# floe/backscrub

Hardware: AMD Instinct MI355X
Metric: composited frames/sec at 640×480 (batch), 1/2/4/8 MI355X + mask IoU vs CPU ref (higher is better)
Workload: dtype f32 (network) / u8 (image kernels); 1 GPU; BASELINE configs[1]: batch=256 640x480 frames, segm_lite_v681.tflite; moving scene: ring of 4 batches, a new one every step; 1 step = prep+network+decode+mask+blend, inputs resident in HBM; streams_per_gpu=256, library=bsx 0.1 (HIP gfx950, f32 NHWC)

## Files before the change

### backscrub_amd/csrc/kernels_seg.hip

```cpp
#ifndef __HIPCC_RTC__
#include <hip/hip_runtime.h>
#endif
#ifndef BSX_SEG_RTC
#include "debug_switches.hpp"

#include <algorithm>
#include <cstdlib>
#include <type_traits>

#include "kernels.hpp"
#include "mfma_tile.hpp"
#include "segments.hpp"
#endif

#if defined(BSX_SEG_RTC)
#define BSX_SEG_D(T, NAME) constexpr T d = kSeg##NAME; (void)d_rt
#elif defined(BSX_SEG_PROBE)
#define BSX_SEG_D(T, NAME) constexpr T d = kProbe##NAME; (void)d_rt
#else
#define BSX_SEG_D(T, NAME) const T& d = d_rt
#endif

namespace bsx {
#ifdef BSX_SEG_RTC
// ... 285 lines not shown
  for (int s = 0; s < 7; s++) {
    const int k = 4 * s + g;
    const bool valid = k < 27;
    const int fy = k / 9, r9 = k - 9 * fy, fx = r9 / 3, ci = r9 - 3 * fx;
    koff[s] = valid ? fy * rowf + fx * 3 + ci : 0;
    ws[s] = valid ? (w + d.stem.w_off)[(unsigned)(k * d.stem.cout_pad + li)] : 0.f;
  }
  const float4 bias_s = ld4(w + d.stem.b_off + cq4);
  const Clamp cl_stem = clamp_of(d.stem.act), cl_pw = clamp_of(d.pw.act), cl_dw = clamp_of(d.dw.act);
  const int ntile = AR * ctiles;
  const int xe = li;
  __syncthreads();

  float* x_f = a_t;
  float wr[4];
  load_wtile(wr, w, d.pw, 0, li, g);
  const float4 bias_p = ld4(w + d.pw.b_off + cq4);
  float4 sumA = f4zero();
  auto stem_pw_epilogue = [&](const f4acc acc, const RowTile rt) {
    float4 v = acc_quad(acc);
    const int x2 = 16 * rt.ct + xe, gy = ar0 + rt.row, gx = ac0 + x2;
    v = f4add(v, bias_s);
    v = STEM_HSWISH ? hswish4(v) : clamp4(v, cl_stem);
    f4acc pa = {0.f, 0.f, 0.f, 0.f};
    if (!(d.dbg_skip & 2)) {
      pa = __builtin_amdgcn_mfma_f32_16x16x4f32(wr[0], v.x, pa, 0, 0, 0);
      pa = __builtin_amdgcn_mfma_f32_16x16x4f32(wr[1], v.y, pa, 0, 0, 0);
      pa = __builtin_amdgcn_mfma_f32_16x16x4f32(wr[2], v.z, pa, 0, 0, 0);
      pa = __builtin_amdgcn_mfma_f32_16x16x4f32(wr[3], v.w, pa, 0, 0, 0);
    }
    if (x2 < AC) {
      const bool row_owned = gy >= max(2 * r0, 0) && gy < min(2 * r0 + 2 * d.TR, d.H1);
      if (row_owned && gx >= 2 * c0 && gx < min(2 * c0 + 2 * d.TC, d.W1)) {
        stg4<H16>(A_out, (unsigned)((gy * d.W1 + gx) * 16 + cq4), v);
        sumA = f4add(sumA, v);
      }
      float4 xv = acc_quad(pa);
      const bool inside = gy >= 0 && gy < d.H1 && gx >= 0 && gx < d.W1;
      xv = inside ? clamp4(f4add(xv, bias_p), cl_pw) : f4zero();
      st4(x_f + (rt.row * AC + x2) * 16 + cq4, xv);
    }
  };
  for (int t = wave; t < ntile && !(d.dbg_skip & 1); t += 8) {
    const bool two = t + 4 < ntile;
    const RowTile r0t = row_tile(t, ctiles, d.m_ct), r1t = row_tile(two ? t + 4 : t, ctiles, d.m_ct);
    const float* base0 = in_t + (2 * r0t.row) * rowf + 6 * min(16 * r0t.ct + li, AC - 1);
    const float* base1 = in_t + (2 * r1t.row) * rowf + 6 * min(16 * r1t.ct + li, AC - 1);
    float av0[7], av1[7];
#pragma unroll
    for (int s7 = 0; s7 < 7; s7++) { av0[s7] = base0[koff[s7]]; av1[s7] = base1[koff[s7]]; }
    f4acc acc0 = {0.f, 0.f, 0.f, 0.f}, acc1 = {0.f, 0.f, 0.f, 0.f};
#pragma unroll
    for (int s7 = 0; s7 < 7; s7++) {
      acc0 = __builtin_amdgcn_mfma_f32_16x16x4f32(ws[s7], av0[s7], acc0, 0, 0, 0);
      acc1 = __builtin_amdgcn_mfma_f32_16x16x4f32(ws[s7], av1[s7], acc1, 0, 0, 0);
    }
    stem_pw_epilogue(acc0, r0t);
    if (two) stem_pw_epilogue(acc1, r1t);
  }
  const int quad = lane & 3, px = lane >> 2;
  f4v wd[9];
#pragma unroll
  for (int k = 0; k < 9; k++) wd[k] = ldv(w + d.dw.w_off + k * 16 + 4 * quad);
  const f4v bias_d = ldv(w + d.dw.b_off + 4 * quad);
  const int cox[3] = {(2 * px) * 16 + 4 * quad, (2 * px + 1) * 16 + 4 * quad, (2 * px + 2) * 16 + 4 * quad};
  __syncthreads();

  float4 sumB = f4zero();
  for (int py = wave; py < d.TR && !(d.dbg_skip & 4); py += 4) {
    if (r0 + py >= d.H2) break;
    if (px < d.TC && c0 + px < d.W2) {
      const float4 v = clamp4(tof4(dw3x3(x_f, AC * 16, 2 * py, cox, wd) + bias_d), cl_dw);
      stg4<H16>(b0_out, (unsigned)(((r0 + py) * d.W2 + c0 + px) * 16 + 4 * quad), v);
      sumB = f4add(sumB, v);
    }
  }
  float* s_red = in_t;
  wave_reduce16<0>(sumA, s_red, wave, lane);
  wave_reduce16<1>(sumB, s_red + 256, wave, lane);
  __syncthreads();
  store_partials(s_red, fa + d.part_a_off + (long)t_ * 16);
  store_partials(s_red + 256, fa + d.part_b0_off + (long)t_ * 16);
}

#ifdef BSX_SEG_RTC
extern "C" __global__ __launch_bounds__(kSegThreads) __attribute__((amdgpu_waves_per_eu(6, 6))) void bsx_seg_k2(
#else
template <bool H16>
__global__ __launch_bounds__(kSegThreads) __attribute__((amdgpu_waves_per_eu(6, 6))) void seg_k2_k(
#endif
    const SegK2 d_rt, float* __restrict__ arena, long per_frame, const float* __restrict__ w, int n_frames) {
  BSX_SEG_D(SegK2, K2);
  unsigned f_, t_;
  xcd_frame_tile((unsigned)(d.tiles_y * d.tiles_x), (unsigned)n_frames, &f_, &t_);
  const int f = (int)f_, ty = (int)t_ / d.tiles_x, tx = (int)t_ - ty * d.tiles_x;
  const int r0 = ty * d.TR, c0 = tx * d.TC;
  const int BR = 2 * d.TR + 1, BC = 2 * d.TC + 1, br0 = 2 * r0 - d.dw_pt, bc0 = 2 * c0 - d.dw_pl, RW = d.rw, ctiles = RW >> 4;
  float* fa = arena + (size_t)f * (size_t)per_frame;
  float* B_t = seg_smem + kScrFloats;
  float* x_t = B_t + BR * RW * 16;
  const float* b0_in = fa + d.b0_off;
  float* B_out = fa + d.B_off;
  float* c0_out = fa + d.c0_off;
  const int tid = threadIdx.x, lane = tid & 63, wave = wave_uniform(tid >> 6), li = lane & 15, g = lane >> 4, cq4 = 4 * g;
  const int ntile = BR * ctiles, xe = li;
  const int la = col_a(li, g), lb = col_b(li, g, RW >> 1);
  constexpr int kB0 = 6;
  float4 b0v[kB0];
#pragma unroll
  for (int j = 0; j < kB0; j++) {
    const int t = wave + 4 * j;
    b0v[j] = f4zero();
    if (t < ntile) {
      const RowTile rt = row_tile(t, ctiles, d.m_ct);
      const int gy = br0 + rt.row, gx = bc0 + 16 * rt.ct + li;
      if (gy >= 0 && gy < d.H2 && gx >= 0 && gx < d.W2) b0v[j] = ldg4<H16>(b0_in, (unsigned)((gy * d.W2 + gx) * 16 + 4 * g));
    }
  }
  seg_gate(d.gate, fa, w, seg_smem, B_t);
  const float4 sv = ld4(seg_smem + kScrGate + 4 * g);
  float wr[4];
  load_wtile(wr, w, d.pw_a, 0, li, g);
  const float4 bias_a = ld4(w + d.pw_a.b_off + cq4);
  const Clamp cl_a = clamp_of(d.pw_a.act), cl_b = clamp_of(d.pw_b.act), cl_dw = clamp_of(d.dw.act);

  float4 sumB = f4zero();
#pragma unroll
  for (int j = 0; j < kB0; j++) {
    const int t = wave + 4 * j;
    if (t >= ntile) break;
    const RowTile rt = row_tile(t, ctiles, d.m_ct);
    float4 a = b0v[j];
    a = make_float4(__fmul_rn(a.x, sv.x), __fmul_rn(a.y, sv.y), __fmul_rn(a.z, sv.z), __fmul_rn(a.w, sv.w));
    const f4acc acc = mma16(a, wr);
    float4 v = acc_quad(acc);
    const int x2 = 16 * rt.ct + xe, hy = br0 + rt.row, hx = bc0 + x2;
    if (x2 < BC) {
      v = clamp4(f4add(v, bias_a), cl_a);
      st4(B_t + (rt.row * RW + 16 * rt.ct) * 16 + la, v);
      const bool row_owned = hy >= max(2 * r0, 0) && hy < min(2 * r0 + 2 * d.TR, d.H2);
      if (row_owned && hx >= 2 * c0 && hx < min(2 * c0 + 2 * d.TC, d.W2)) {
        stg4<H16>(B_out, (unsigned)((hy * d.W2 + hx) * 16 + cq4), v);
        sumB = f4add(sumB, v);
      }
    }
  }
  float* s_red = seg_smem + kScrRed;
  wave_reduce16<0>(sumB, s_red, wave, lane);
  __syncthreads();
  store_partials(s_red, fa + d.part_B_off + (long)t_ * 16);

  const int C = d.dw.C, ngrp = (C + 15) >> 4, quad = lane & 3, px = lane >> 2;
  const int cox[3] = {col_b(2 * px, quad, RW >> 1), col_b(2 * px + 1, quad, RW >> 1), col_b(2 * px + 2, quad, RW >> 1)};
  for (int grp = 0; grp < ngrp && !(d.dbg_skip & 2); grp++) {
    load_wtile(wr, w, d.pw_b, 16 * grp, li, g);
    const float4 bias_b = ld4(w + d.pw_b.b_off + 16 * grp + cq4);
    for (int t = wave; t < ntile; t += 4) {
      const RowTile rt = row_tile(t, ctiles, d.m_ct);
      const f4acc acc = mma16(ld4(B_t + (rt.row * RW + 16 * rt.ct) * 16 + la), wr);
      float4 v = acc_quad(acc);
      const int x2 = 16 * rt.ct + xe, hy = br0 + rt.row, hx = bc0 + x2;
      if (x2 < BC) {
        const bool inside = hy >= 0 && hy < d.H2 && hx >= 0 && hx < d.W2;
        v = inside ? clamp4(f4add(v, bias_b), cl_b) : f4zero();
        st4(x_t + (rt.row * RW + 8 * rt.ct) * 16 + lb, v);
      }
    }
    const int ch = 16 * grp + 4 * quad;
    f4v wd[9];
    f4v bias_d = {0.f, 0.f, 0.f, 0.f};
    if (ch < C) {
#pragma unroll
      for (int k = 0; k < 9; k++) wd[k] = ldv(w + d.dw.w_off + (unsigned)(k * C + ch));
      bias_d = ldv(w + d.dw.b_off + ch);
    }
    __syncthreads();
    if (ch < C && px < d.TC && c0 + px < d.W3)
      for (int py = wave; py < d.TR && r0 + py < d.H3; py += 4) {
        const float4 v = clamp4(tof4(dw3x3(x_t, RW * 16, 2 * py, cox, wd) + bias_d), cl_dw);
        stg4<H16>(c0_out, (unsigned)(((r0 + py) * d.W3 + c0 + px) * C + ch), v);
      }
    __syncthreads();
  }
}

constexpr int kGatedRows = 5;
constexpr int kLoStride = kSegLoStride;
struct GatedPre { float4 s[kGatedRows]; int ly0, lx0, LC; };
template <bool H16>
__device__ __forceinline__ GatedPre gated_prefetch(const float* __restrict__ skip, const float* __restrict__ lo, int H, int W, int HL, int WL, bool half_pixel,
                                                   float hs, float wsc, int r0, int c0, int ZH, int ZC, float* l_t) {
  const int tid = threadIdx.x, lane = tid & 63, wave = wave_uniform(tid >> 6), li = lane & 15, g = lane >> 4;
  GatedPre pre;
  const int ix = c0 - 1 + li;
  const bool col_in = li < ZC && ix >= 0 && ix < W;
#pragma unroll
  for (int j = 0; j < kGatedRows; j++) {
    const int zy = wave + 4 * j, iy = r0 - 1 + zy;
    pre.s[j] = f4zero();
    if (zy < ZH && iy >= 0 && iy < H && col_in) pre.s[j] = ldg4<H16>(skip, (unsigned)((iy * W + ix) * 16 + 4 * g));
  }
  int ly0, ly1, lx0, lx1, t0, t1;
  float fr;
  up_axis(max(r0 - 1, 0), hs, half_pixel, HL, &ly0, &t1, &fr);
  up_axis(min(r0 - 2 + ZH, H - 1), hs, half_pixel, HL, &t0, &ly1, &fr);
  up_axis(max(c0 - 1, 0), wsc, half_pixel, WL, &lx0, &t1, &fr);
  up_axis(min(c0 - 2 + ZC, W - 1), wsc, half_pixel, WL, &t0, &lx1, &fr);
  const int LR = ly1 - ly0 + 1, LC = lx1 - lx0 + 1;
  pre.ly0 = ly0; pre.lx0 = lx0; pre.LC = LC;
  float4 v[3];
#pragma unroll
  for (int j = 0; j < 3; j++) {
    const int ly = wave + 4 * j;
    v[j] = f4zero();
    if (ly < LR && lane < LC * 4) v[j] = ldg4<H16>(lo, (unsigned)(((ly0 + ly) * WL + lx0 + (lane >> 2)) * 16 + 4 * (lane & 3)));
  }
#pragma unroll
  for (int j = 0; j < 3; j++) {
    const int ly = wave + 4 * j;
    if (ly < LR && lane < LC * 4) st4(l_t + ly * LC * kLoStride + col_l(lane >> 2, lane & 3), v[j]);
  }
  return pre;
}
__device__ __forceinline__ void gated_compute(const GatedPre& pre, const float* l_t, int H, int W, int HL, int WL, bool half_pixel, float hs, float wsc, const float* s_gate,
                                              const SegConvW& pw, const float* __restrict__ w, int r0, int c0, int ZH, int ZC, float* z_t) {
  const int tid = threadIdx.x, lane = tid & 63, wave = wave_uniform(tid >> 6), li = lane & 15, g = lane >> 4, cq4 = 4 * g;
  float wr[4];
  load_wtile(wr, w, pw, 0, li, g);
  const float4 bias = ld4(w + pw.b_off + cq4);
  const float4 gv = ld4(s_gate + 4 * g);
  const Clamp cl = clamp_of(pw.act);
  const int ix = c0 - 1 + li;
  int x0, x1;
  float dx;
  up_axis(min(max(ix, 0), W - 1), wsc, half_pixel, WL, &x0, &x1, &dx);
  const int xo0 = col_l(x0 - pre.lx0, g), xo1 = col_l(x1 - pre.lx0, g);
  const int xe = li;
  const bool ecol_in = xe < ZC && ix >= 0 && ix < W;
#pragma unroll
  for (int j = 0; j < kGatedRows; j++) {
    const int zy = wave + 4 * j, iy = r0 - 1 + zy;
    if (zy >= ZH) break;
    const bool row_in = iy >= 0 && iy < H;
    int y0, y1;
    float dy;
    up_axis(min(max(iy, 0), H - 1), hs, half_pixel, HL, &y0, &y1, &dy);
    const float* l0 = l_t + (y0 - pre.ly0) * pre.LC * kLoStride;
    const float* l1 = l_t + (y1 - pre.ly0) * pre.LC * kLoStride;
    const float4 ta = ld4(l0 + xo0), tb = ld4(l1 + xo0), tc = ld4(l0 + xo1), td = ld4(l1 + xo1);
    const float w00 = (1.f - dy) * (1.f - dx), w10 = dy * (1.f - dx), w01 = (1.f - dy) * dx, w11 = dy * dx;
    const float4 sk = pre.s[j];
    float4 a;
    a.x = fmaf(sk.x, gv.x, fmaf(td.x, w11, fmaf(tc.x, w01, fmaf(tb.x, w10, ta.x * w00))));
    a.y = fmaf(sk.y, gv.y, fmaf(td.y, w11, fmaf(tc.y, w01, fmaf(tb.y, w10, ta.y * w00))));
    a.z = fmaf(sk.z, gv.z, fmaf(td.z, w11, fmaf(tc.z, w01, fmaf(tb.z, w10, ta.z * w00))));
    a.w = fmaf(sk.w, gv.w, fmaf(td.w, w11, fmaf(tc.w, w01, fmaf(tb.w, w10, ta.w * w00))));
    const f4acc acc = mma16(a, wr);
    float4 v = acc_quad(acc);
    v = (ecol_in && row_in) ? clamp4(f4add(v, bias), cl) : f4zero();
    if (xe < ZC) st4(z_t + zy * 256 + col_a(xe, g), v);
  }
}

#ifdef BSX_SEG_RTC
extern "C" __global__ __launch_bounds__(kSegThreads) void bsx_seg_k3(
#else
template <bool H16>
__global__ __launch_bounds__(kSegThreads) void seg_k3_k(
#endif
    const SegK3 d_rt, float* __restrict__ arena, long per_frame, const float* __restrict__ w, int n_frames) {
  BSX_SEG_D(SegK3, K3);
  unsigned f_, t_;
  xcd_frame_tile((unsigned)(d.tiles_y * d.tiles_x), (unsigned)n_frames, &f_, &t_);
  const int f = (int)f_, ty = (int)t_ / d.tiles_x, tx = (int)t_ - ty * d.tiles_x;
  const int r0 = ty * d.TR, c0 = tx * d.TC, ZH = d.TR + 2, ZC = d.TC + 2;
  float* fa = arena + (size_t)f * (size_t)per_frame;
  float* z_t = seg_smem + kScrFloats;
  float* l_t = z_t + ZH * 256;
  float* lo_out = fa + d.lo_off;
  const int tid = threadIdx.x, lane = tid & 63, wave = wave_uniform(tid >> 6), li = lane & 15, g = lane >> 4, cq4 = 4 * g;
  const GatedPre pre = gated_prefetch<H16>(fa + d.skip_off, fa + d.lo2_off, d.H2, d.W2, d.HL, d.WL, d.half_pixel != 0, d.hs, d.ws, r0, c0, ZH, ZC, l_t);
  if (tid < 16) seg_smem[kScrGate + tid] = fa[d.g_off + tid];
  __syncthreads();
  gated_compute(pre, l_t, d.H2, d.W2, d.HL, d.WL, d.half_pixel != 0, d.hs, d.ws, seg_smem + kScrGate, d.pw1, w, r0, c0, ZH, ZC, z_t);
  const int pc = min(li, 13);
  const int coz[3] = {col_a(pc, g), col_a(pc + 1, g), col_a(pc + 2, g)};
  f4v wd[9];
#pragma unroll
  for (int k = 0; k < 9; k++) wd[k] = ldv(w + d.dw.w_off + k * 16 + cq4);
  const f4v bias_d = ldv(w + d.dw.b_off + cq4);
  const Clamp cl_dw = clamp_of(d.dw.act), cl_2 = clamp_of(d.pw2.act);
  float wr[4];
  load_wtile(wr, w, d.pw2, 0, li, g);
  const float4 bias2 = ld4(w + d.pw2.b_off + cq4);
  __syncthreads();
  float4 sum = f4zero();
  const int xe = li;
  for (int py = wave; py < d.TR && r0 + py < d.H2; py += 4) {
    const f4v zc = ldv(z_t + (py + 1) * 256 + coz[1]);
    const float4 dv = clamp4(tof4(dw3x3(z_t, 256, py, coz, wd) + bias_d), cl_dw);
    const f4acc acc = mma16(f4add(dv, tof4(zc)), wr);
    float4 v = acc_quad(acc);
    if (xe < d.TC && c0 + xe < d.W2) {
      v = clamp4(f4add(v, bias2), cl_2);
      stg4<H16>(lo_out, (unsigned)(((r0 + py) * d.W2 + c0 + xe) * 16 + cq4), v);
      sum = f4add(sum, v);
    }
  }
  float* s_red = seg_smem + kScrRed;
  wave_reduce16<0>(sum, s_red, wave, lane);
  __syncthreads();
  store_partials(s_red, fa + d.part_lo_off + (long)t_ * 16);
}

#ifdef BSX_SEG_RTC
extern "C" __global__ __launch_bounds__(kSegThreads) __attribute__((amdgpu_waves_per_eu(5, 5))) void bsx_seg_tail(
#else
template <int CO, bool LOGITS, bool SIGMOID, bool H16>
__global__ __launch_bounds__(kSegThreads) __attribute__((amdgpu_waves_per_eu(5, 5))) void seg_tail_k(
#endif
    const SegTail d_rt, float* __restrict__ arena, long per_frame, float* __restrict__ net_out,
                                                          uint8_t* __restrict__ ofinal, const float* __restrict__ w, int n_frames, const int* __restrict__ slot_of) {
  BSX_SEG_D(SegTail, TAIL);
  unsigned f_, t_;
  xcd_frame_tile((unsigned)(d.tiles_y * d.tiles_x), (unsigned)n_frames, &f_, &t_);
  const int f = (int)f_, ty = (int)t_ / d.tiles_x, tx = (int)t_ - ty * d.tiles_x;
  const int r0 = ty * d.TR, c0 = tx * d.TC, ZH = d.TR + 2, ZC = d.TC + 2;
  float* fa = arena + (size_t)f * (size_t)per_frame;
  float* z_t = seg_smem + kScrFloats;
  float* l_t = z_t + max(ZH * 256, kGateStageFloats);
  uint8_t* of = ofinal + (size_t)(slot_of ? slot_of[f] : f) * (size_t)(d.H0 * d.W0);
  float* no = net_out + (size_t)f * (size_t)(d.H0 * d.W0 * CO);
  const int tid = threadIdx.x, lane = tid & 63, wave = wave_uniform(tid >> 6), li = lane & 15, g = lane >> 4, cq4 = 4 * g;
  const int fy = g >> 1, fx = g & 1, ix = c0 + li;
  const GatedPre pre = gated_prefetch<H16>(fa + d.skip_off, fa + d.lo_off, d.H1, d.W1, d.HL, d.WL, d.half_pixel != 0, d.hs, d.ws, r0, c0, ZH, ZC, l_t);
  constexpr int kRowsB = 5;
// ... 143 lines not shown
```

### backscrub_amd/csrc/plan.cpp

```cpp
#include "debug_switches.hpp"
#include "plan.hpp"
#include "gen_seg.hpp"
#include "gen_mid.hpp"

#include <algorithm>
#include <cmath>
#include <cstdio>
#include <cstdlib>
#include <cstring>
#include <map>

namespace bsx {
namespace {

void conv_geometry(int in, int k, int s, int d, bool same, int* out, int* pad) {
  int eff = (k - 1) * d + 1;
  *out = same ? (in + s - 1) / s : (in + s - eff) / s;
  int total = (*out - 1) * s + eff - in;
  *pad = total > 0 ? total / 2 : 0;
}

uint16_t f32_to_f16_rn(float f) {
  uint32_t x; memcpy(&x, &f, 4);
  const uint32_t sign = (x >> 16) & 0x8000u;
// ... 445 lines not shown
      if ((m.kind == (int)StepKind::PwConv && m.gemv) || m.kind == kMicroTail || m.kind == (int)StepKind::Conv) return;
    lower_frame_program(g, plan, steps, ext, part_n, part_hw, 64, policy);
    if (plan->program.empty()) lower_frame_program(g, plan, steps, ext, part_n, part_hw, kLdsScratchFloats, policy);
  };
  if (const char* force = BSX_DBG_ENV("BSX_PLAN_POLICY")) { plan->program_policy = (unsigned)atoi(force) & 7u; lower(plan->program_policy); plan->program_arena_bytes = program_arena_bytes(*plan); return; }
  unsigned best = 0;
  long best_b = -1;
  for (unsigned pol = 0; pol < 8; pol++) {
    lower(pol);
    if (plan->program.empty()) continue;
    const long b = program_arena_bytes(*plan);
    if (best_b < 0 || b < best_b) { best_b = b; best = pol; }
  }
  lower(best);
  plan->program_policy = best;
  plan->program_arena_bytes = program_arena_bytes(*plan);
}

std::string verify_program_lds(const Plan& plan) {
  const auto& b = plan.program_blocks;
  for (size_t i = 0; i < b.size(); i++) {
    if (b[i].off < plan.program_scratch_floats || b[i].off + b[i].len > plan.lds_zero_off() || b[i].len <= 0 || b[i].from > b[i].until)
      return "block out of range: " + b[i].what;
    for (size_t j = i + 1; j < b.size(); j++) {
      const bool time = b[i].from <= b[j].until && b[j].from <= b[i].until;
      const bool mem = b[i].off < b[j].off + b[j].len && b[j].off < b[i].off + b[i].len;
      if (time && mem) return "overlap: " + b[i].what + " [" + std::to_string(b[i].from) + "," + std::to_string(b[i].until) + "] and " + b[j].what + " [" +
                              std::to_string(b[j].from) + "," + std::to_string(b[j].until) + "]";
    }
  }
  for (const MicroOp& m : plan.program) {
    for (const Loc* l : {&m.in0, &m.in1, &m.in2, &m.res, &m.scale, &m.out})
      if (l->space == kLocLds && (l->off < plan.program_scratch_floats || l->off >= plan.program_lds_floats)) return "operand outside the LDS block area";
    if (m.stage_floats > 0 && (m.w_lds < plan.program_scratch_floats || m.w_lds + m.stage_floats > plan.program_lds_floats)) return "weight slot outside the LDS block area";
  }
  return "ok";
}


namespace {

bool resize_weights_uniform(int in, int out, bool align, bool half_pixel) {
  std::vector<double> wsum(in, 0.0);
  const float scale = (align && out > 1) ? (float)(in - 1) / (float)(out - 1) : (float)in / (float)out;
  for (int o = 0; o < out; o++) {
    const float v = half_pixel ? ((float)o + 0.5f) * scale - 0.5f : (float)o * scale;
    const float fl = std::floor(v);
    const int lo = std::max((int)fl, 0), hi = std::min((int)std::ceil(v), in - 1);
    const float frac = v - (float)lo;
    wsum[lo] += 1.0 - frac; wsum[hi] += frac;
  }
  const double want = (double)out / (double)in;
  for (double x : wsum) if (std::fabs(x - want) > 1e-5) return false;
  return true;
}

SegConvW conv_w(const Step& st) { SegConvW c; c.w_off = (long long)st.w_off; c.b_off = (long long)st.b_off; c.Cin = st.kh * st.kw * st.Cin; c.Cout = st.Cout; c.cout_pad = st.cout_pad; c.act = st.act; return c; }
SegDwW dw_w(const Step& st) { SegDwW c; c.w_off = (long long)st.w_off; c.b_off = (long long)st.b_off; c.C = st.Cout; c.act = st.act; return c; }
SegFc fc_w(const Step& st) { SegFc c; c.w_off = (long long)st.w2_off; c.b_off = (long long)st.b_off; c.Cin = st.Cin; c.Cout = st.Cout; c.act = st.act; return c; }

bool is_pw16(const Step& st) { return st.kind == StepKind::PwConv && st.Cin == 16 && st.Cout == 16 && st.cout_pad == 16 && st.OH * st.OW > 4; }
bool is_fc_step(const Step& st) { return st.kind == StepKind::PwConv && st.OH * st.OW == 1 && st.w2_off != 0 && st.residual < 0 && st.in_scale < 0 && st.in2 < 0 && st.Cin <= 32 && st.Cin % 8 == 0 && st.Cout <= 32; }
bool is_dw3(const Step& st, int stride) {
  return st.kind == StepKind::DwConv && st.kh == 3 && st.kw == 3 && st.sh == stride && st.sw == stride && st.dh == 1 && st.dw == 1;
}
int tiles_for(int extent, int target) { return (extent + target - 1) / target; }

}

static bool seg_fail(int where) { if (BSX_DBG_ENV("BSX_SEG_DEBUG")) fprintf(stderr, "segmentation: check %d failed\n", where); return false; }
static bool build_segments(Graph& g, Plan* plan) {
  const std::vector<Step>& S = plan->steps;
  const int NS = (int)S.size();
  if (NS < 9 + 15) return seg_fail(1);
  auto uses_of = [&](int t) {
    int n = 0;
    for (const Step& q : S) {
      for (int u : {q.concat_in.empty() ? q.in0 : -1, q.in1, q.in2, q.residual, q.in_scale}) n += (u == t);
      for (int u : q.concat_in) n += (u == t);
    }
    return n + (t == g.output);
  };
  auto dims = [&](int t, int k) { return g.tensors[t].dims[k]; };

  const Step &stem = S[0], &hpw = S[1], &hdw = S[2];
  if (!(stem.kind == StepKind::Conv && stem.in0 == g.input && stem.kh == 3 && stem.kw == 3 && stem.sh == 2 && stem.sw == 2 && stem.dh == 1 && stem.dw == 1 &&
        stem.Cin == 3 && stem.Cout == 16 && stem.cout_pad == 16 && stem.residual < 0)) return seg_fail(2);
  const int A = stem.out;
  if (!(is_pw16(hpw) && hpw.in0 == A && hpw.residual < 0 && hpw.in_scale < 0 && hpw.in2 < 0 && uses_of(hpw.out) == 1)) return seg_fail(3);
  if (!(is_dw3(hdw, 2) && hdw.in0 == hpw.out && hdw.Cout == 16 && hdw.residual < 0)) return seg_fail(4);
  const int b0 = hdw.out;
  const Step &g1 = S[3], &f1a = S[4], &f1b = S[5], &pwa = S[6], &pwb = S[7], &kdw = S[8];
  if (!(g1.kind == StepKind::Gap && g1.concat_in.empty() && g1.in0 == b0 && is_fc_step(f1a) && f1a.in0 == g1.out && is_fc_step(f1b) && f1b.in0 == f1a.out &&
        f1a.Cin == 16 && f1b.Cout == 16 && uses_of(b0) == 2)) return seg_fail(5);
  if (!(is_pw16(pwa) && pwa.in0 == b0 && pwa.in_scale == f1b.out && pwa.residual < 0 && pwa.in2 < 0 && uses_of(f1b.out) == 1)) return seg_fail(6);
  const int B = pwa.out;
  if (!(pwb.kind == StepKind::PwConv && pwb.in0 == B && pwb.Cin == 16 && pwb.cout_pad % 16 == 0 && pwb.residual < 0 && pwb.in_scale < 0 && pwb.in2 < 0 &&
        uses_of(pwb.out) == 1 && pwb.Cout % 4 == 0)) return seg_fail(7);
  if (!(is_dw3(kdw, 2) && kdw.in0 == pwb.out && kdw.residual < 0)) return seg_fail(8);
  const int c0 = kdw.out;
  const Step &tr = S[NS - 7], &tg = S[NS - 6], &tf1 = S[NS - 5], &tf2 = S[NS - 4], &tpw = S[NS - 3], &tdw = S[NS - 2], &ttc = S[NS - 1];
  if (!(tr.kind == StepKind::Resize && tr.Cin == 16 && tr.OH == dims(A, 1) && tr.OW == dims(A, 2))) return seg_fail(9);
  const int lo = tr.in0, up = tr.out;
  auto pools = [](const Step& q, int a, int b) { return q.kind == StepKind::Gap && q.concat_in.size() == 2 && ((q.concat_in[0] == a && q.concat_in[1] == b) || (q.gap_sum && q.concat_in[0] == b && q.concat_in[1] == a)); };
  if (!(pools(tg, A, up) && is_fc_step(tf1) && tf1.in0 == tg.out &&
        is_fc_step(tf2) && tf2.in0 == tf1.out && tf2.Cout == 16)) return seg_fail(10);
  if (!(is_pw16(tpw) && tpw.in0 == A && tpw.in_scale == tf2.out && tpw.in2 == up && tpw.residual < 0)) return seg_fail(11);
  if (!(is_dw3(tdw, 1) && tdw.in0 == tpw.out && tdw.residual == tpw.out && tdw.Cout == 16 && tdw.pad_t == 1 && tdw.pad_l == 1)) return seg_fail(12);
  if (!(ttc.kind == StepKind::TConv && ttc.in0 == tdw.out && ttc.kh == 2 && ttc.kw == 2 && ttc.Cin == 16 && (ttc.Cout == 1 || ttc.Cout == 2) && ttc.out == g.output)) return seg_fail(13);
  if (uses_of(A) != 3 || uses_of(up) != 2 || uses_of(tpw.out) != 2 || uses_of(tdw.out) != 1 || uses_of(tf2.out) != 1) return seg_fail(14);
  if (!resize_weights_uniform(tr.H, tr.OH, tr.align_corners, tr.half_pixel) || !resize_weights_uniform(tr.W, tr.OW, tr.align_corners, tr.half_pixel)) return seg_fail(15);
  const Step &kr = S[NS - 14], &kg = S[NS - 13], &kf1 = S[NS - 12], &kf2 = S[NS - 11], &kp1 = S[NS - 10], &kd = S[NS - 9], &kp2 = S[NS - 8];
  if (!(kr.kind == StepKind::Resize && kr.Cin == 16 && kr.OH == dims(B, 1) && kr.OW == dims(B, 2))) return seg_fail(16);
  const int lo2 = kr.in0, up2 = kr.out;
  if (!(pools(kg, B, up2) && is_fc_step(kf1) && kf1.in0 == kg.out &&
        is_fc_step(kf2) && kf2.in0 == kf1.out && kf2.Cout == 16)) return seg_fail(17);
  if (!(is_pw16(kp1) && kp1.in0 == B && kp1.in_scale == kf2.out && kp1.in2 == up2 && kp1.residual < 0)) return seg_fail(18);
  if (!(is_dw3(kd, 1) && kd.in0 == kp1.out && kd.residual == kp1.out && kd.Cout == 16 && kd.pad_t == 1 && kd.pad_l == 1)) return seg_fail(19);
  if (!(is_pw16(kp2) && kp2.in0 == kd.out && kp2.out == lo && kp2.residual < 0 && kp2.in_scale < 0 && kp2.in2 < 0)) return seg_fail(20);
  if (uses_of(B) != 3 || uses_of(up2) != 2 || uses_of(kp1.out) != 2 || uses_of(kd.out) != 1 || uses_of(kf2.out) != 1 || uses_of(lo) != 1 || uses_of(lo2) != 1) return seg_fail(21);
  if (!resize_weights_uniform(kr.H, kr.OH, kr.align_corners, kr.half_pixel) || !resize_weights_uniform(kr.W, kr.OW, kr.align_corners, kr.half_pixel)) return seg_fail(22);
  if (uses_of(c0) != 1) return seg_fail(23);
  auto clampish = [](int a) { return a == kActNone || a == kActRelu || a == kActRelu6; };
  if (!(clampish(stem.act) || stem.act == kActHswish) || !(ttc.act == kActNone || ttc.act == kActSigmoid) || (ttc.act == kActSigmoid && ttc.Cout != 1)) return seg_fail(34);
  for (const Step* q : {&hpw, &hdw, &pwa, &pwb, &kdw, &kp1, &kd, &kp2, &tpw, &tdw}) if (!clampish(q->act)) return seg_fail(35);

  size_t top = plan->arena_floats_per_stream;
  auto reserve = [&](size_t floats) { size_t at = top; top += (floats + 63) / 64 * 64; return (long long)at; };
  auto synth = [&](const char* name, int n, int C) {
    TensorInfo t; t.dims[0] = 1; t.dims[1] = n; t.dims[2] = 1; t.dims[3] = C; t.shape = {1, n, 1, C}; t.name = name;
    g.tensors.push_back(t);
    plan->tensor_off.push_back(-1);
    return (int)g.tensors.size() - 1;
  };
  SegPlan sp;
  int tgt[8] = {4, 14, 4, 7, 16, 14, 18, 14};
  if (const char* e = BSX_DBG_ENV("BSX_SEG_TILES")) sscanf(e, "%d,%d,%d,%d,%d,%d,%d,%d", &tgt[0], &tgt[1], &tgt[2], &tgt[3], &tgt[4], &tgt[5], &tgt[6], &tgt[7]);
  auto split = [&](int extent, int target, int* tile, int* n) { *n = tiles_for(extent, std::max(1, target)); *tile = (extent + *n - 1) / *n; };

  SegHead& h = sp.head;
  h.H0 = stem.H; h.W0 = stem.W; h.H1 = stem.OH; h.W1 = stem.OW; h.H2 = hdw.OH; h.W2 = hdw.OW;
  h.stem_pt = stem.pad_t; h.stem_pl = stem.pad_l; h.dw_pt = hdw.pad_t; h.dw_pl = hdw.pad_l;
  h.stem = conv_w(stem); h.pw = conv_w(hpw); h.dw = dw_w(hdw);
  split(h.H2, tgt[0], &h.TR, &h.tiles_y); split(h.W2, tgt[1], &h.TC, &h.tiles_x);
  h.lds_floats = seg_head_lds_floats(h);
  h.rw = seg_row_width(2 * h.TC + 1); h.m_ct = (65536u + (unsigned)(h.rw / 16) - 1) / (unsigned)(h.rw / 16);
  if (h.TR > 4 || h.TC > 15 || (4 * h.TC + 3) * 3 > 192) return seg_fail(30);
  SegK2& k2 = sp.k2;
  k2.H2 = hdw.OH; k2.W2 = hdw.OW; k2.H3 = kdw.OH; k2.W3 = kdw.OW; k2.dw_pt = kdw.pad_t; k2.dw_pl = kdw.pad_l;
  k2.pw_a = conv_w(pwa); k2.pw_b = conv_w(pwb); k2.dw = dw_w(kdw);
  split(k2.H3, tgt[2], &k2.TR, &k2.tiles_y); split(k2.W3, tgt[3], &k2.TC, &k2.tiles_x);
  k2.lds_floats = seg_k2_lds_floats(k2);
  k2.rw = seg_row_width(2 * k2.TC + 1); k2.m_ct = (65536u + (unsigned)(k2.rw / 16) - 1) / (unsigned)(k2.rw / 16);
  if (k2.TC > 15 || ((2 * k2.TR + 1) * (k2.rw / 16) + 3) / 4 > 6) return seg_fail(31);
  SegK3& k3 = sp.k3;
  k3.H2 = kp1.OH; k3.W2 = kp1.OW; k3.HL = kr.H; k3.WL = kr.W; k3.half_pixel = kr.half_pixel; k3.align_corners = kr.align_corners;
  k3.pw1 = conv_w(kp1); k3.pw2 = conv_w(kp2); k3.dw = dw_w(kd);
  split(k3.H2, tgt[4], &k3.TR, &k3.tiles_y); split(k3.W2, tgt[5], &k3.TC, &k3.tiles_x);
  k3.hs = seg_up_scale(k3.HL, k3.H2, k3.align_corners != 0); k3.ws = seg_up_scale(k3.WL, k3.W2, k3.align_corners != 0);
  if (!BSX_DBG_ENV("BSX_SEG_LO_WORST")) k3.lo_floats = seg_lo_window_floats(k3.H2, k3.W2, k3.HL, k3.WL, k3.half_pixel != 0, k3.align_corners != 0, k3.TR, k3.TC, k3.tiles_y, k3.tiles_x);
  k3.lds_floats = seg_k3_lds_floats(k3);
  if (k3.TC > 14 || k3.TR > 18) return seg_fail(32);
  SegTail& tl = sp.tail;
  tl.H1 = tpw.OH; tl.W1 = tpw.OW; tl.HL = tr.H; tl.WL = tr.W; tl.H0 = ttc.OH; tl.W0 = ttc.OW; tl.half_pixel = tr.half_pixel; tl.align_corners = tr.align_corners;
  tl.pw = conv_w(tpw); tl.dw = dw_w(tdw); tl.tc_w_off = (long long)ttc.w_off; tl.tc_b_off = (long long)ttc.b_off; tl.Co = ttc.Cout; tl.act3 = ttc.act;
  split(tl.H1, tgt[6], &tl.TR, &tl.tiles_y); split(tl.W1, tgt[7], &tl.TC, &tl.tiles_x);
  tl.hs = seg_up_scale(tl.HL, tl.H1, tl.align_corners != 0); tl.ws = seg_up_scale(tl.WL, tl.W1, tl.align_corners != 0);
  if (!BSX_DBG_ENV("BSX_SEG_LO_WORST")) tl.lo_floats = seg_lo_window_floats(tl.H1, tl.W1, tl.HL, tl.WL, tl.half_pixel != 0, tl.align_corners != 0, tl.TR, tl.TC, tl.tiles_y, tl.tiles_x);
  tl.lds_floats = seg_tail_lds_floats(tl);
  if (tl.TC > 14 || tl.TR > 18) return seg_fail(33);
  const int lds_cap = 160 * 256;
  if (h.lds_floats > lds_cap || k2.lds_floats > lds_cap || k3.lds_floats > lds_cap || tl.lds_floats > lds_cap) return seg_fail(24);
  if (ttc.OH != 2 * tpw.OH || ttc.OW != 2 * tpw.OW || h.H2 != k3.H2 || h.W2 != k3.W2) return seg_fail(25);
  if (h.tiles_y * h.tiles_x > 1024 || k2.tiles_y * k2.tiles_x > 1024 || k3.tiles_y * k3.tiles_x > 1024) return seg_fail(26);

  const int pA = synth("partials(A)", h.tiles_y * h.tiles_x, 16), pb0 = synth("partials(b0)", h.tiles_y * h.tiles_x, 16);
  const int pB = synth("partials(B)", k2.tiles_y * k2.tiles_x, 16), plo = synth("partials(lo)", k3.tiles_y * k3.tiles_x, 16);
  const int pgt = BSX_DBG_ENV("BSX_SEG_NO_GATE_KERNEL") ? -1 : synth("gate(tail)", 1, 16);
  if (pgt >= 0) plan->tensor_off[pgt] = reserve(16);
  for (int t : {A, b0, B, c0, lo2, lo, kf2.out, pA, pb0, pB, plo}) plan->tensor_off[t] = reserve(g.tensors[t].elems());
  for (int t : {hpw.out, g1.out, f1a.out, f1b.out, pwb.out, up2, kg.out, kf1.out, kp1.out, kd.out, up, tg.out, tf1.out, tf2.out, tpw.out, tdw.out})
    if (t != g.output) plan->tensor_off[t] = -1;
  plan->arena_floats_per_stream = top;
  plan->seg_stored = {A, b0, B, c0, lo};

  h.a_off = plan->tensor_off[A]; h.b0_off = plan->tensor_off[b0]; h.part_a_off = plan->tensor_off[pA]; h.part_b0_off = plan->tensor_off[pb0];
  k2.b0_off = plan->tensor_off[b0]; k2.B_off = plan->tensor_off[B]; k2.c0_off = plan->tensor_off[c0]; k2.part_B_off = plan->tensor_off[pB];
  k2.gate.n_parts = 1; k2.gate.n_fc = 2; k2.gate.sum_parts = 0;
  k2.gate.part[0].off = plan->tensor_off[pb0]; k2.gate.part[0].n = h.tiles_y * h.tiles_x; k2.gate.part[0].C = 16; k2.gate.part[0].hw = (float)(h.H2 * h.W2);
  k2.gate.fc[0] = fc_w(f1a); k2.gate.fc[1] = fc_w(f1b);
  k3.skip_off = plan->tensor_off[B]; k3.lo2_off = plan->tensor_off[lo2]; k3.g_off = plan->tensor_off[kf2.out]; k3.lo_off = plan->tensor_off[lo];
  k3.part_lo_off = plan->tensor_off[plo];
  tl.skip_off = plan->tensor_off[A]; tl.lo_off = plan->tensor_off[lo];
  tl.gate.n_parts = 2; tl.gate.n_fc = 2; tl.gate.sum_parts = tg.gap_sum ? 1 : 0;
  tl.gate.part[0].off = plan->tensor_off[pA]; tl.gate.part[0].n = h.tiles_y * h.tiles_x; tl.gate.part[0].C = 16; tl.gate.part[0].hw = (float)(h.H1 * h.W1);
  tl.gate.part[1].off = plan->tensor_off[plo]; tl.gate.part[1].n = k3.tiles_y * k3.tiles_x; tl.gate.part[1].C = 16; tl.gate.part[1].hw = (float)(k3.H2 * k3.W2);
  tl.gate.fc[0] = fc_w(tf1); tl.gate.fc[1] = fc_w(tf2);
  if (BSX_DBG_ENV("BSX_SEG_GATE_SKIP")) k2.gate.timing_skip = tl.gate.timing_skip = 1;
  if (const char* e = BSX_DBG_ENV("BSX_SEG_SKIP")) sscanf(e, "%d,%d,%d,%d", &h.dbg_skip, &k2.dbg_skip, &k3.dbg_skip, &tl.dbg_skip);
  tl.pre_gate_off = pgt >= 0 ? plan->tensor_off[pgt] : -1;
  if (tl.gate.fc[0].Cin != (tl.gate.sum_parts ? 16 : 32) || k2.gate.fc[0].Cin != 16) return seg_fail(27);

  std::vector<Step> mid(S.begin() + 9, S.begin() + (NS - 14));
  Step gate = kg;
  gate.concat_in = {B, lo2};
  gate.in0 = B;
  gate.label += "*";
  mid.push_back(gate); mid.push_back(kf1); mid.push_back(kf2);
  std::map<int, int> part_n, part_hw;
  part_n[B] = k2.tiles_y * k2.tiles_x; part_hw[B] = k2.H2 * k2.W2;
  const long B_real = plan->tensor_off[B];
  plan->tensor_off[B] = plan->tensor_off[pB];
  build_frame_program(g, plan, mid, {c0, B, lo2, kf2.out}, part_n, part_hw);
  plan->tensor_off[B] = B_real;
  if (plan->program.empty()) return seg_fail(28);
  sp.on = true;
  plan->seg = sp;
#ifdef BSX_DEBUG_SWITCHES
  if (const char* path = BSX_DBG_ENV("BSX_SEG_DUMP")) {
    if (FILE* f = fopen(path, "w")) { fputs(seg_constants_text(sp, "kProbe").c_str(), f); fclose(f); }
  }
#endif
  char line[256];
  plan->seg_text.clear();
  auto add = [&](const char* name, int TR, int TC, int ty, int tx, int lds, std::initializer_list<int> stores) {
    snprintf(line, sizeof line, "segment %-5s tile %dx%d, %dx%d tiles per frame, LDS %.1f KiB, stores", name, TR, TC, ty, tx, lds / 256.0);
    plan->seg_text += line;
    for (int t : stores) plan->seg_text += " t" + std::to_string(t);
    plan->seg_text += stores.size() ? "\n" : " the network output\n";
  };
  add("head", h.TR, h.TC, h.tiles_y, h.tiles_x, h.lds_floats, {A, b0}); add("k2", k2.TR, k2.TC, k2.tiles_y, k2.tiles_x, k2.lds_floats, {B, c0});
  add("k3", k3.TR, k3.TC, k3.tiles_y, k3.tiles_x, k3.lds_floats, {lo}); add("tail", tl.TR, tl.TC, tl.tiles_y, tl.tiles_x, tl.lds_floats, {});
  return true;
}


MidGeometry mid_geometry_default() {
  static const MidGeometry geo = [] {
    MidGeometry m{kFrameThreads, kLdsTotalFloats};
    if (const char* e = BSX_DBG_ENV("BSX_MID_LANES")) { const int v = atoi(e); if (v == 512 || v == 1024) m.lanes = v; }
    if (const char* e = BSX_DBG_ENV("BSX_MID_LDS_KB")) { const int v = atoi(e); if (v >= 64 && v <= 160) m.lds_floats = v * 256; }
    return m;
  }();
  return geo;
}

bool build_plan(const Graph& g_in, Plan* plan, std::string* err, bool reuse_arena, bool segments) {
  auto fail = [&](const std::string& m) { if (err) *err = m; return false; };
  { const MidGeometry geo = mid_geometry_default(); plan->mid_lanes = geo.lanes; plan->lds_total_floats = geo.lds_floats; }
  Graph g = g_in;
  int NT = (int)g.tensors.size();
  const int NN = (int)g.nodes.size();

  std::vector<std::vector<int>> users(NT);
  for (int i = 0; i < NN; i++) for (int t : g.nodes[i].inputs) if (t >= 0 && !g.tensors[t].is_const) users[t].push_back(i);
  auto single_user = [&](int t) -> int { return (t != g.output && users[t].size() == 1) ? users[t][0] : -1; };

  std::vector<char> fused(NN, 0);
  std::vector<Step> steps;
  std::vector<float>& W = plan->weights;
  W.clear();
  auto align_w = [&]() { while (W.size() % 4) W.push_back(0.f); };

  for (int i = 0; i < NN; i++) {
    if (fused[i]) continue;
    const Node& n = g.nodes[i];
    const TensorInfo& out_t = g.tensors[n.output];
    Step st;
    st.last_node = n.index;
    auto T = [&](int k) -> const TensorInfo& { return g.tensors[n.inputs[k]]; };

    auto chain_epilogue = [&](int cur) -> int {
      for (;;) {
        int u = single_user(cur);
        if (u < 0 || fused[u]) break;
        const Node& y = g.nodes[u];
        if (is_unary(y.type) && st.act == kActNone && st.residual < 0) {
          st.act = unary_act(y.type); fused[u] = 1; cur = y.output; st.last_node = y.index; continue;
        }
        if (y.type == OpType::Add && y.act == kActNone && st.residual < 0 && y.inputs.size() == 2) {
          int other = y.inputs[0] == cur ? y.inputs[1] : y.inputs[0];
          if (other >= 0 && other != cur && !g.tensors[other].is_const && same_dims(g.tensors[other], g.tensors[cur])) {
            st.residual = other; fused[u] = 1; cur = y.output; st.last_node = y.index; continue;
          }
        }
        break;
      }
      return cur;
    };

    switch (n.type) {
      case OpType::Conv:
      case OpType::FullyConnected: {
        if (n.inputs.size() < 2) return fail("conv without weights");
        const TensorInfo& x = T(0);
        const TensorInfo& w = T(1);
        if (!w.is_const) return fail("non-constant conv weights unsupported");
        const TensorInfo* b = (n.inputs.size() > 2 && n.inputs[2] >= 0) ? &T(2) : nullptr;
        if (b && !b->is_const) return fail("non-constant bias unsupported");
        bool fc = n.type == OpType::FullyConnected;
        st.in0 = n.inputs[0];
        st.H = x.dims[1]; st.W = x.dims[2]; st.Cin = x.dims[3];
        if (fc) {
          st.Cout = w.dims[2]; st.kh = st.kw = 1;
          if (w.dims[3] != st.Cin) return fail("FULLY_CONNECTED depth mismatch");
          st.OH = st.H; st.OW = st.W;
        } else {
          st.Cout = w.dims[0]; st.kh = w.dims[1]; st.kw = w.dims[2];
          if (w.dims[3] != st.Cin) return fail("CONV_2D depth mismatch");
          st.sh = n.stride_h; st.sw = n.stride_w; st.dh = n.dil_h; st.dw = n.dil_w;
          conv_geometry(st.H, st.kh, st.sh, st.dh, n.same_padding, &st.OH, &st.pad_t);
          conv_geometry(st.W, st.kw, st.sw, st.dw, n.same_padding, &st.OW, &st.pad_l);
        }
        if (st.OH != out_t.dims[1] || st.OW != out_t.dims[2] || st.Cout != out_t.dims[3]) return fail("conv output shape mismatch at op #" + std::to_string(n.index));
        bool pw = st.kh == 1 && st.kw == 1 && st.sh == 1 && st.sw == 1;
        st.kind = pw ? StepKind::PwConv : StepKind::Conv;
        st.act = n.act;
        if (pw) {
          int prod = -1;
          for (int j = 0; j < i; j++) if (!fused[j] && g.nodes[j].output == st.in0) prod = j;
          if (prod >= 0 && g.nodes[prod].type == OpType::Mul && g.nodes[prod].act == kActNone && single_user(st.in0) == i) {
            const Node& m = g.nodes[prod];
            int a = m.inputs[0], s2 = m.inputs[1];
            if (a >= 0 && s2 >= 0 && !g.tensors[a].is_const && !g.tensors[s2].is_const) {
              if (is_chan_vec(g.tensors[a], g.tensors[s2])) std::swap(a, s2);
              if (is_chan_vec(g.tensors[s2], g.tensors[a])) {
                for (size_t k = 0; k < steps.size(); k++)
                  if (steps[k].kind == StepKind::Eltwise && steps[k].out == st.in0) { steps.erase(steps.begin() + k); break; }
                st.in0 = a; st.in_scale = s2;
              }
            }
          }
        }
        int ct = st.Cout <= 16 ? 16 : 32;
        if (!pw) ct = 16;
        st.cout_tile = ct;
        st.cout_pad = round_up(st.Cout, ct);
        align_w();
        st.w_off = W.size();
        W.resize(W.size() + (size_t)st.kh * st.kw * st.Cin * st.cout_pad, 0.f);
        for (int o = 0; o < st.Cout; o++) for (int fy = 0; fy < st.kh; fy++) for (int fx = 0; fx < st.kw; fx++) for (int c = 0; c < st.Cin; c++) {
          size_t src = fc ? ((size_t)o * st.Cin + c) : ((((size_t)o * st.kh + fy) * st.kw + fx) * st.Cin + c);
          W[st.w_off + (((size_t)fy * st.kw + fx) * st.Cin + c) * st.cout_pad + o] = w.f32[src];
        }
        align_w();
        st.b_off = W.size();
        W.resize(W.size() + st.cout_pad, 0.f);
        if (b) for (int o = 0; o < st.Cout; o++) W[st.b_off + o] = b->f32[o];
        if (pw && st.OH * st.OW <= 4 && st.Cin % 4 == 0) {
          align_w();
          st.w2_off = W.size();
          W.resize(W.size() + (size_t)st.Cout * st.Cin);
// ... 424 lines not shown
```

### backscrub_amd/csrc/segments.hpp

```cpp
#pragma once
#ifndef BSX_SEG_RTC
#include <algorithm>
#include <cmath>
#include <cstdint>
#endif

namespace bsx {

struct SegConvW { long long w_off = 0, b_off = 0; int Cin = 0, Cout = 0, cout_pad = 0, act = 0; };
struct SegDwW { long long w_off = 0, b_off = 0; int C = 0, act = 0; };
struct SegFc { long long w_off = 0, b_off = 0; int Cin = 0, Cout = 0, act = 0; };
struct SegPart { long long off = 0; int n = 0, C = 0; float hw = 1.f; };
struct SegGate {
  int n_parts = 0, sum_parts = 0, n_fc = 0;
  int timing_skip = 0;
  SegPart part[2];
  SegFc fc[2];
};

constexpr int kSegThreads = 256;
constexpr int kSegMaxC = 16;

struct SegHead {
  int H0 = 0, W0 = 0, H1 = 0, W1 = 0, H2 = 0, W2 = 0;
  int stem_pt = 0, stem_pl = 0, dw_pt = 0, dw_pl = 0;
  SegConvW stem, pw;
  SegDwW dw;
  long long a_off = 0, b0_off = 0, part_a_off = 0, part_b0_off = 0;
  int TR = 0, TC = 0, tiles_y = 0, tiles_x = 0;
  int lds_floats = 0;
  int dbg_skip = 0;
  int rw = 0;
  unsigned m_ct = 0;
};

struct SegK2 {
  int H2 = 0, W2 = 0, H3 = 0, W3 = 0;
  int dw_pt = 0, dw_pl = 0;
  SegGate gate;
  SegConvW pw_a, pw_b;
  SegDwW dw;
  long long b0_off = 0, B_off = 0, c0_off = 0, part_B_off = 0;
  int TR = 0, TC = 0, tiles_y = 0, tiles_x = 0;
  int lds_floats = 0;
  int dbg_skip = 0;
  int rw = 0;
  unsigned m_ct = 0;
};

struct SegK3 {
  int H2 = 0, W2 = 0, HL = 0, WL = 0;
  int half_pixel = 0, align_corners = 0;
  SegConvW pw1, pw2;
  SegDwW dw;
  long long skip_off = 0, lo2_off = 0, g_off = 0, lo_off = 0, part_lo_off = 0;
  int TR = 0, TC = 0, tiles_y = 0, tiles_x = 0;
  int lds_floats = 0;
  int lo_floats = 0;
  float hs = 0.f, ws = 0.f;
  int dbg_skip = 0;
};

struct SegTail {
  int H1 = 0, W1 = 0, HL = 0, WL = 0, H0 = 0, W0 = 0;
  int half_pixel = 0, align_corners = 0;
  SegGate gate;
  SegConvW pw;
  SegDwW dw;
  long long tc_w_off = 0, tc_b_off = 0;
  int Co = 0, act3 = 0, model_type = 0;
  long long skip_off = 0, lo_off = 0;
  long long pre_gate_off = -1;
  int TR = 0, TC = 0, tiles_y = 0, tiles_x = 0;
  int lds_floats = 0;
  int lo_floats = 0;
  float hs = 0.f, ws = 0.f;
  int dbg_skip = 0;
};

constexpr int kSegLoStride = 16;
constexpr int kSegLoTileFloats = 12 * 16 * kSegLoStride;
constexpr int kSegScratchFloats = 640;
constexpr int kSegGateStageFloats = 512 + 2 * (32 * 32 + 32);
#ifndef BSX_SEG_RTC
inline int seg_row_width(int cols) { return (cols + 15) / 16 * 16; }
inline int seg_head_lds_floats(const SegHead& d) {
  const int AR = 2 * d.TR + 1, AC = 2 * d.TC + 1, IR = 2 * AR + 1, IC = 2 * AC + 1;
  const int win = (IR * IC * 3 + 3) & ~3;
  return (win > 512 ? win : 512) + AR * AC * 16;
}
inline int seg_k2_lds_floats(const SegK2& d) { const int v = 2 * (2 * d.TR + 1) * seg_row_width(2 * d.TC + 1) * 16; return kSegScratchFloats + (v > kSegGateStageFloats ? v : kSegGateStageFloats); }
inline void seg_up_axis(int o, float scale, bool half_pixel, int in_size, int* lo, int* hi) {
  const float v = half_pixel ? ((float)o + 0.5f) * scale + -0.5f : (float)o * scale;
  const float fl = std::floor(v);
  *lo = std::max((int)fl, 0);
  *hi = std::min((int)std::ceil(v), in_size - 1);
}
inline float seg_up_scale(int in, int out, bool align) { return (align && out > 1) ? (float)(in - 1) / (float)(out - 1) : (float)in / (float)out; }
inline int seg_lo_window_floats(int H, int W, int HL, int WL, bool half_pixel, bool align, int TR, int TC, int tiles_y, int tiles_x) {
  const float hs = seg_up_scale(HL, H, align), ws = seg_up_scale(WL, W, align);
  int lr = 1, lc = 1, a, b, c, e;
  for (int ty = 0; ty < tiles_y; ty++) {
    const int r0 = ty * TR;
    seg_up_axis(std::max(r0 - 1, 0), hs, half_pixel, HL, &a, &b);
    seg_up_axis(std::min(r0 + TR, H - 1), hs, half_pixel, HL, &c, &e);
    lr = std::max(lr, e - a + 1);
  }
  for (int tx = 0; tx < tiles_x; tx++) {
    const int c0 = tx * TC;
    seg_up_axis(std::max(c0 - 1, 0), ws, half_pixel, WL, &a, &b);
    seg_up_axis(std::min(c0 + TC, W - 1), ws, half_pixel, WL, &c, &e);
    lc = std::max(lc, e - a + 1);
  }
  const int need = (lr + 1) * (lc + 1) * kSegLoStride;
  return need < kSegLoTileFloats ? need : kSegLoTileFloats;
}
inline int seg_k3_lds_floats(const SegK3& d) { return kSegScratchFloats + (d.TR + 2) * 256 + (d.lo_floats > 0 ? d.lo_floats : kSegLoTileFloats); }
inline int seg_tail_lds_floats(const SegTail& d) { const int v = (d.TR + 2) * 256; return kSegScratchFloats + (v > kSegGateStageFloats ? v : kSegGateStageFloats) + (d.lo_floats > 0 ? d.lo_floats : kSegLoTileFloats); }
#endif

struct SegPlan {
  bool on = false;
  SegHead head;
  SegK2 k2;
  SegK3 k3;
  SegTail tail;
};

}
```

Baseline: 720,600 frames/s.

## Give each wave a private 3-row staging buffer in k2 to drop block barriers

```diff
diff --git a/backscrub_amd/csrc/kernels_seg.hip b/backscrub_amd/csrc/kernels_seg.hip
--- a/backscrub_amd/csrc/kernels_seg.hip
+++ b/backscrub_amd/csrc/kernels_seg.hip
@@ -461,7 +461,44 @@
 
   const int C = d.dw.C, ngrp = (C + 15) >> 4, quad = lane & 3, px = lane >> 2;
   const int cox[3] = {col_b(2 * px, quad, RW >> 1), col_b(2 * px + 1, quad, RW >> 1), col_b(2 * px + 2, quad, RW >> 1)};
-  for (int grp = 0; grp < ngrp && !(d.dbg_skip & 2); grp++) {
+  float* x_w = x_t + wave * (3 * RW * 16);
+  const int py = wave;
+  for (int grp = 0; grp < ngrp && !(d.dbg_skip & (2 | 16)) && py < d.TR && r0 + py < d.H3; grp++) {
+    load_wtile(wr, w, d.pw_b, 16 * grp, li, g);
+    const float4 bias_b = ld4(w + d.pw_b.b_off + 16 * grp + cq4);
+    const int ch = 16 * grp + 4 * quad;
+    f4v wd[9];
+    f4v bias_d = {0.f, 0.f, 0.f, 0.f};
+    if (ch < C) {
+#pragma unroll
+      for (int k = 0; k < 9; k++) wd[k] = ldv(w + d.dw.w_off + (unsigned)(k * C + ch));
+      bias_d = ldv(w + d.dw.b_off + ch);
+    }
+    int rwf = RW * 16;
+#ifndef BSX_SEG_RTC
+    asm volatile("" : "+s"(rwf));
+#endif
+    for (int ct = 0; ct < ctiles; ct++) {
+      const int x2 = 16 * ct + xe, hx = bc0 + x2;
+#pragma unroll
+      for (int r = 0; r < 3; r++) {
+        float4 v = acc_quad(mma16(ld4(B_t + (2 * py + r) * rwf + 256 * ct + la), wr));
+        const int hy = br0 + 2 * py + r;
+        if (x2 < BC) {
+          const bool inside = hy >= 0 && hy < d.H2 && hx >= 0 && hx < d.W2;
+          v = inside ? clamp4(f4add(v, bias_b), cl_b) : f4zero();
+          st4(x_w + r * rwf + 128 * ct + lb, v);
+        }
+      }
+    }
+    asm volatile("" ::: "memory");
+    if (ch < C && px < d.TC && c0 + px < d.W3) {
+      const float4 v = clamp4(tof4(dw3x3(x_w, rwf, 0, cox, wd) + bias_d), cl_dw);
+      stg4<H16>(c0_out, (unsigned)(((r0 + py) * d.W3 + c0 + px) * C + ch), v);
+    }
+  }
+#if defined(BSX_SEG_RTC) || defined(BSX_DEBUG_SWITCHES)
+  for (int grp = 0; grp < ngrp && (d.dbg_skip & (2 | 16)) == 16; grp++) {
     load_wtile(wr, w, d.pw_b, 16 * grp, li, g);
     const float4 bias_b = ld4(w + d.pw_b.b_off + 16 * grp + cq4);
     for (int t = wave; t < ntile; t += 4) {
@@ -491,6 +528,7 @@
       }
     __syncthreads();
   }
+#endif
 }
 
 constexpr int kGatedRows = 5;
diff --git a/backscrub_amd/csrc/plan.cpp b/backscrub_amd/csrc/plan.cpp
--- a/backscrub_amd/csrc/plan.cpp
+++ b/backscrub_amd/csrc/plan.cpp
@@ -621,7 +621,7 @@
   split(k2.H3, tgt[2], &k2.TR, &k2.tiles_y); split(k2.W3, tgt[3], &k2.TC, &k2.tiles_x);
   k2.lds_floats = seg_k2_lds_floats(k2);
   k2.rw = seg_row_width(2 * k2.TC + 1); k2.m_ct = (65536u + (unsigned)(k2.rw / 16) - 1) / (unsigned)(k2.rw / 16);
-  if (k2.TC > 15 || ((2 * k2.TR + 1) * (k2.rw / 16) + 3) / 4 > 6) return seg_fail(31);
+  if (k2.TR > 4 || k2.TC > 15 || ((2 * k2.TR + 1) * (k2.rw / 16) + 3) / 4 > 6) return seg_fail(31);
   SegK3& k3 = sp.k3;
   k3.H2 = kp1.OH; k3.W2 = kp1.OW; k3.HL = kr.H; k3.WL = kr.W; k3.half_pixel = kr.half_pixel; k3.align_corners = kr.align_corners;
   k3.pw1 = conv_w(kp1); k3.pw2 = conv_w(kp2); k3.dw = dw_w(kd);
@@ -667,6 +667,7 @@
   tl.gate.fc[0] = fc_w(tf1); tl.gate.fc[1] = fc_w(tf2);
   if (BSX_DBG_ENV("BSX_SEG_GATE_SKIP")) k2.gate.timing_skip = tl.gate.timing_skip = 1;
   if (const char* e = BSX_DBG_ENV("BSX_SEG_SKIP")) sscanf(e, "%d,%d,%d,%d", &h.dbg_skip, &k2.dbg_skip, &k3.dbg_skip, &tl.dbg_skip);
+  if (BSX_DBG_ENV("BSX_SEG_K2_SHARED")) k2.dbg_skip |= 16;
   tl.pre_gate_off = pgt >= 0 ? plan->tensor_off[pgt] : -1;
   if (tl.gate.fc[0].Cin != (tl.gate.sum_parts ? 16 : 32) || k2.gate.fc[0].Cin != 16) return seg_fail(27);
 
diff --git a/backscrub_amd/csrc/segments.hpp b/backscrub_amd/csrc/segments.hpp
--- a/backscrub_amd/csrc/segments.hpp
+++ b/backscrub_amd/csrc/segments.hpp
@@ -89,7 +89,11 @@
   const int win = (IR * IC * 3 + 3) & ~3;
   return (win > 512 ? win : 512) + AR * AC * 16;
 }
-inline int seg_k2_lds_floats(const SegK2& d) { const int v = 2 * (2 * d.TR + 1) * seg_row_width(2 * d.TC + 1) * 16; return kSegScratchFloats + (v > kSegGateStageFloats ? v : kSegGateStageFloats); }
+inline int seg_k2_lds_floats(const SegK2& d) {
+  const int BR = 2 * d.TR + 1, xr = 3 * (kSegThreads / 64);
+  const int v = (BR + (xr > BR ? xr : BR)) * seg_row_width(2 * d.TC + 1) * 16;
+  return kSegScratchFloats + (v > kSegGateStageFloats ? v : kSegGateStageFloats);
+}
 inline void seg_up_axis(int o, float scale, bool half_pixel, int in_size, int* lo, int* hi) {
   const float v = half_pixel ? ((float)o + 0.5f) * scale + -0.5f : (float)o * scale;
   const float fl = std::floor(v);
```

Measured after the change: 727,200 frames/s, median of 6. No clear change (+0.9%).
